# ricklisz/AnatoMask

Hardware: AMD Instinct MI355X
Metric: pretrain volumes/sec @128^3 patch mask=0.6 (higher is better)
Workload: dtype bf16; 1 GPU; STUNet-B AnatoMask step, 128^3 patch, mask_ratio 0.6, bf16 storage/MFMA + fp32 master; per_gpu_batch=16, global_batch=16, parallelism=dp1, step=teacher fwd + sampler + student fwd + loss + bwd + clip + AdamW + EMA

## Files before the change

### anatomask_amd/csrc/conv_igemm.hip

```cpp
#include <mutex>
#include <type_traits>
#include <stdlib.h>
#include "common.h"
#include "../../include/anatomask_hip.h"
#include "conv_plan.h"

using namespace amconv;

namespace {

template <typename T, int BD, int BH, int BW, int NS, int NIT, int TGS = 3, bool HR = false, bool NB = false, bool HT = false>
__global__ __launch_bounds__(256, (TGS == 2 && BD * BH * BW <= 256) ? 3 : 2) void conv_igemm_kernel(ConvArgs a) {
  constexpr int EPC = TT<T>::EPC;
  constexpr bool SPL = std::is_same<T, f32s_t>::value;
  constexpr int KC = (ROWB / 16) * EPC;
  constexpr int MV = BD * BH * BW;
  constexpr int VS = MV / 64;
  constexpr int NT = 16 * NS;
  constexpr int TG = TG_OF(NS, TGS);
  constexpr int WBUF = TG * NT * ROWB;
  constexpr int WCH = TG * NT * 4;
  constexpr int WIT = (WCH + 255) / 256;
  static_assert(MV % 64 == 0, "brick must give each wave whole 16-voxel subtiles");
  extern __shared__ __attribute__((aligned(16))) unsigned char lds[];
// ... 416 lines not shown
#pragma unroll
    for (int i = 0; i < NS; ++i)
#pragma unroll
      for (int r = 0; r < 4; ++r) {
        float s1 = 0.f, s2 = 0.f;
#pragma unroll
        for (int j = 0; j < VS; ++j) { const float o = acc[i][j][r]; s1 += o; s2 += o * o; }
        if (!AM_DBG(a, 2048)) { s1 = row16_sum(s1); s2 = row16_sum(s2); }
        if (r16 == 0) {
          const int c = (i >> 1) * 32 + g * 8 + (i & 1) * 4 + r;
          red[(wave * 16 * NS + c) * 2] = s1; red[(wave * 16 * NS + c) * 2 + 1] = s2;
        }
      }
    if (!AM_DBG(a, 1024)) __syncthreads();
    if (tid < 16 * NS && co0 + tid < a.Cout) {
      float s1 = 0.f, s2 = 0.f;
#pragma unroll
      for (int w = 0; w < 4; ++w) { s1 += red[(w * 16 * NS + tid) * 2]; s2 += red[(w * 16 * NS + tid) * 2 + 1]; }
      part[(co0 + tid) * 2] = s1; part[(co0 + tid) * 2 + 1] = s2;
    }
  }
}

template <typename T, int BD, int BH, int BW, int NS, int NIT, int TGS = 3, bool HR = false, bool NB = false, bool HT = false>
int launch(Plan& P, hipStream_t st) {
  ConvArgs& a = P.a;
  constexpr auto kern = conv_igemm_kernel<T, BD, BH, BW, NS, NIT, TGS, HR, NB, HT>;
  if (P.lds > 160 * 1024) return -3;
  AM_HIP_STAGE(am_lds_optin<kern>());
  const unsigned nbrick = a.plist ? (unsigned)a.nlive : (unsigned)(a.B * a.nbd * a.nbh * a.nbw);
  a.ny = (a.Cout + 16 * NS - 1) / (16 * NS);
  const unsigned nsib = (unsigned)(a.ny * a.nclass);
  dim3 grid(nsib > 1 ? ((nbrick + 7) / 8) * 8 * nsib : nbrick, 1, 1);
  AM_LAUNCH(kern, grid, dim3(256), P.lds, st, a);
  AM_CHECK_LAUNCH_STAGE();
  return 1;
}

template <typename T, int NS>
int dispatch_nit(Plan& P, int shape, hipStream_t st) {
  const int n = P.nit;
  if (P.a.nb_x) {
    if constexpr (sizeof(T) == 2) {
      if (P.tgs != 3 || P.a.OS != 1) return -7;
      if (shape == 2) return n <= 4 ? launch<T, 4, 4, 4, NS, 4, 3, false, true>(P, st) : -7;
      if (shape == 1) return n > 7 && n <= 11 ? (P.a.hreuse ? launch<T, 4, 4, 16, NS, 11, 3, true, true>(P, st) : launch<T, 4, 4, 16, NS, 11, 3, false, true>(P, st)) : -7;
// ... 54 lines not shown
  const int qd = (p.Do + os - 1) / os, qh = (p.Ho + os - 1) / os, qw = (p.Wo + os - 1) / os; const bool out_sparse = p.out_sparse;
  bool big_ok = p.dtype == AM_DT_BF16;
#ifdef AM_ABLATE
  { const char* e_ = getenv("AM_CV_NOBIG"); if (e_ && atoi(e_)) big_ok = false; }
#endif
  int shape = brick_shape(os, qh, qw, out_sparse, p.out_bshift, bd, bh, bw);
  *nt = Cout <= 32 ? 32 : 64;
  const long q = (long)qd * qh * qw;
  auto nwg = [&](int tile) { return (long)B * ((qd + *bd - 1) / *bd) * ((qh + *bh - 1) / *bh) * ((qw + *bw - 1) / *bw) * ((Cout + tile - 1) / tile) * (os == 2 ? 8 : 1); };
  if (nwg(*nt) < 256) {
    *nt = 32;
    if (nwg(32) < 192 && shape != 2) { shape = 2; *bh = 4; *bw = 4; }
  }
  if (os == 2 && !out_sparse && shape == 1 && *nt == 64 && qh >= 8 && nwg(64) >= 4096 && big_ok) { shape = 3; *bh = 8; }
  return shape;
}

extern "C" int am_packed_dims(int dtype, int rows, int k, int* rows_padded, int* k_padded) {
  const int tile = rows <= 32 ? 32 : 64;
  const int kc = dtype == AM_DT_BF16 ? 32 : 16;
  *rows_padded = (rows + tile - 1) / tile * tile;
  *k_padded = (k + kc - 1) / kc * kc;
  return 0;
}

int amconv::conv_igemm_fits(const ConvProblem& p) {
  const int os = p.mode == AM_CONV_DGRAD ? p.stride : (p.mode == AM_CONVT_FWD ? 2 : 1);
  int bd, bh, bw, nt;
  pick_tiling(p, &bd, &bh, &bw, &nt);
  return p.B * ((p.Do + os * bd - 1) / (os * bd)) * ((p.Ho + os * bh - 1) / (os * bh)) * ((p.Wo + os * bw - 1) / (os * bw)) * (os == 2 ? 8 : 1);
}

bool amconv::conv_igemm_serves(const ConvProblem& p) { return !p.prenorm; }

int amconv::conv_igemm_launch(const ConvProblem& p, ConvArgs& a0, const int* active_list, void* stream, int* rows) {
  if (!conv_igemm_serves(p)) return 0;
  Plan P;
  ConvArgs& a = P.a = a0;
  const int shape = pick_tiling(p, &P.bd, &P.bh, &P.bw, &P.nt_tile);
  const int rc = build_plan(P, p.mode, p.ksize, p.stride);
  if (rc) return rc;
  if (a.OS == 2 && p.accumulate && !p.partials && a.tap_begin[1] > a.tap_begin[0] && a.tap_begin[8] == a.tap_begin[1]) a.nclass = 1;
  if ((size_t)24 * p.Hi * p.Wi * p.Cin * 4 >= 0x7fffff00ull) return -5;
  const int Qd = (p.Do + a.OS - 1) / a.OS, Qh = (p.Ho + a.OS - 1) / a.OS, Qw = (p.Wo + a.OS - 1) / a.OS;
  a.nbd = (Qd + P.bd - 1) / P.bd; a.nbh = (Qh + P.bh - 1) / P.bh; a.nbw = (Qw + P.bw - 1) / P.bw;
  {
    const int qblock = p.out_sparse ? ((1 << p.out_bshift) / a.OS) : 0;
    a.brick_in_patch = qblock > 0 && qblock % P.bd == 0 && qblock % P.bh == 0 && qblock % P.bw == 0;
    bool listed = a.brick_in_patch && active_list && p.n_active > 0 && p.fd <= 255 && p.fh <= 255 && p.fw <= 255 && p.B <= 255 &&
                  Qd == p.fd * qblock && Qh == p.fh * qblock && Qw == p.fw * qblock;
#ifdef AM_ABLATE
    { const char* e = getenv("AM_CV_NOLIST"); if (e && atoi(e)) listed = false; }
#endif
    if (listed) {
      a.plist = active_list; a.pbd = qblock / P.bd; a.pbh = qblock / P.bh; a.pbw = qblock / P.bw;
      a.nlive = p.n_active * a.pbd * a.pbh * a.pbw;
    }
  }
  if (p.partials && p.dtype == AM_DT_BF16) {
    const size_t tile = (size_t)P.bd * P.bh * P.bw * (P.nt_tile * 2 + 32);
    if (P.lds < tile) P.lds = tile;
  }
  if (p.nbred) {
    const size_t tiles = (size_t)P.bd * P.bh * P.bw * (P.nt_tile * 4 + 32);
    if (P.lds < tiles) P.lds = tiles;
  }
  a.nt_store = ((size_t)p.B * p.Do * p.Ho * p.Wo * p.Cout * 2 >= ((size_t)384 << 20) && !p.accumulate) || AM_DBG(a, 8);
  hipStream_t st = (hipStream_t)stream;
  if (rows) *rows = (a.plist ? a.nlive : a.B * a.nbd * a.nbh * a.nbw) * a.nclass;
  return p.dtype == AM_DT_BF16 ? dispatch<bf16_t>(P, shape, st) : p.dtype == AM_DT_F32S ? dispatch<f32s_t>(P, shape, st) : dispatch<float>(P, shape, st);
}

#define AM_STAGE_ROW(name_) {#name_, name_##_fits, name_##_serves, name_##_launch}
static const ConvStage conv_stages[] = {AM_STAGE_ROW(conv_k3t), AM_STAGE_ROW(conv_k3), AM_STAGE_ROW(conv_rw), AM_STAGE_ROW(conv_gather), AM_STAGE_ROW(conv_igemm)};

static void query_masks(ConvProblem& p, bool sparse, int in_bshift, int out_bshift, int n_active) {
  p.in_sparse = p.out_sparse = sparse; p.same_mask = p.has_list = true;
  p.in_bshift = in_bshift; p.out_bshift = out_bshift; p.n_active = n_active;
}

extern "C" int am_conv3d_partials_rows(int mode, int dtype, int ksize, int stride, int B, int Do, int Ho, int Wo, int Cin, int Cout, int out_sparse,
                                       int out_bshift, int n_active, int* rows) {
  ConvProblem p{mode, dtype, ksize, stride, B, Do, Ho, Wo, Cin, Do, Ho, Wo, Cout};
  query_masks(p, out_sparse != 0, out_bshift, out_bshift, n_active);
  *rows = 0;
  for (const ConvStage& s : conv_stages) { const int r = s.fits(p); if (r > *rows) *rows = r; }
  return 0;
}

extern "C" int am_conv3d_uses_k3(int mode, int dtype, int ksize, int stride, int B, int Di, int Hi, int Wi, int Cin, int Do, int Ho, int Wo, int Cout,
                                 int has_masks, int accumulate, int fused_epilogue, int want_partials) {
  ConvProblem p{mode, dtype, ksize, stride, B, Di, Hi, Wi, Cin, Do, Ho, Wo, Cout};
  query_masks(p, has_masks != 0, 0, 0, 0);
  p.accumulate = accumulate != 0; p.ep = fused_epilogue != 0; p.partials = want_partials != 0;
  for (const ConvStage& s : conv_stages)
    if (s.serves(p)) return s.launch == conv_k3t_launch ? 2 : s.launch == conv_k3_launch ? 1 : 0;
  return 0;
}

static ConvArgs fill_args(const ConvProblem& p, const void* x, const void* w_packed, const float* bias, void* y, float* partials, const uint8_t* in_mask,
                          int in_bshift, const uint8_t* out_mask, int out_bshift, int fd, int fh, int fw, int accumulate) {
  ConvArgs a{};
  a.x = x; a.w = w_packed; a.bias = bias; a.y = y; a.partials = partials;
  a.B = p.B; a.Di = p.Di; a.Hi = p.Hi; a.Wi = p.Wi; a.Cin = p.Cin; a.Do = p.Do; a.Ho = p.Ho; a.Wo = p.Wo; a.Cout = p.Cout;
  am_packed_dims(p.dtype, p.Cout, p.Cin, &a.Coutp, &a.Cinp);
  a.w_bytes = p.ksize * p.ksize * p.ksize * a.Coutp * a.Cinp * (p.dtype == AM_DT_BF16 ? 2 : 4);
  a.in_mask = MaskView{in_mask, fd, fh, fw, in_bshift};
  a.out_mask = MaskView{out_mask, fd, fh, fw, out_bshift};
  a.accumulate = accumulate & 1; a.stats_sum_only = (accumulate & AM_CONV_PARTIALS_SUM_ONLY) ? 1 : 0;
#ifdef AM_ABLATE
  { const char* e = getenv("AM_CV_DBG"); a.dbg = e ? atoi(e) : 0; }
#endif
  return a;
}

static int conv3d_impl(ConvProblem& p, ConvArgs& a, const int* active_list, int n_active, void* stream, int* rows) {
  if (p.Cin % 8 || p.Cout % 8) return -1;
  p.in_sparse = a.in_mask.m != nullptr; p.out_sparse = a.out_mask.m != nullptr; p.same_mask = a.in_mask.m == a.out_mask.m;
  p.in_bshift = a.in_mask.bs; p.out_bshift = a.out_mask.bs; p.fd = a.in_mask.fd; p.fh = a.in_mask.fh; p.fw = a.in_mask.fw;
  p.has_list = active_list != nullptr; p.n_active = n_active;
  p.accumulate = a.accumulate != 0; p.sum_only = a.stats_sum_only != 0; p.partials = a.partials != nullptr;
  p.ep = a.ep_scale || a.ep_res || a.ep_act != AM_ACT_NONE; p.nbred = a.nb_x != nullptr; p.prenorm = a.in_scale != nullptr;
  for (const ConvStage& s : conv_stages) {
    const int rc = s.launch(p, a, active_list, stream, rows);
    if (rc) return rc == 1 ? 0 : rc;
  }
  return -7;
}

extern "C" int am_conv3d(int mode, int dtype, int ksize, int stride, const void* x, const void* w_packed,
                         const float* bias, void* y, int B, int Di, int Hi, int Wi, int Cin, int Do, int Ho, int Wo,
                         int Cout, const uint8_t* in_mask, int in_bshift, const uint8_t* out_mask, int out_bshift,
                         int fd, int fh, int fw, int accumulate, float* partials, const float* ep_scale, const float* ep_shift,
                         const void* ep_res, int ep_act, const int32_t* active_list, int n_active, int* partial_rows_written,
                         void* stream) {
  if (ep_scale && !ep_shift) return -1;
  ConvProblem p{mode, dtype, ksize, stride, B, Di, Hi, Wi, Cin, Do, Ho, Wo, Cout};
  ConvArgs a = fill_args(p, x, w_packed, bias, y, partials, in_mask, in_bshift, out_mask, out_bshift, fd, fh, fw, accumulate);
  a.ep_scale = ep_scale; a.ep_shift = ep_scale ? ep_shift : nullptr; a.ep_res = ep_res; a.ep_act = ep_act;
  return conv3d_impl(p, a, active_list, n_active, stream, partial_rows_written);
}

extern "C" int am_conv3d_prenorm_supported(int mode, int dtype, int ksize, int stride, int B, int Do, int Ho, int Wo, int Cin, int Cout,
                                           int sparse, int in_bshift, int out_bshift, int n_active) {
  if (!sparse) return 0;
// ... 8 lines not shown
                                 int out_bshift, int fd, int fh, int fw, float* partials, const float* in_scale, const float* in_shift,
                                 int in_act, const int32_t* active_list, int n_active, int* partial_rows_written, void* stream) {
  if (!in_scale || !in_shift || !mask || !active_list) return -1;
  if (in_act != AM_ACT_NONE && in_act != AM_ACT_LRELU && in_act != AM_ACT_RELU6) return -1;
  ConvProblem p{mode, dtype, ksize, stride, B, Di, Hi, Wi, Cin, Do, Ho, Wo, Cout};
  ConvArgs a = fill_args(p, x, w_packed, bias, y, partials, mask, in_bshift, mask, out_bshift, fd, fh, fw, 0);
  a.in_scale = in_scale; a.in_shift = in_shift; a.in_act = in_act;
  return conv3d_impl(p, a, active_list, n_active, stream, partial_rows_written);
}

extern "C" int am_conv3d_nbred(int mode, int dtype, int ksize, int stride, const void* x, const void* w_packed, void* y, int B, int Di,
                               int Hi, int Wi, int Cin, int Do, int Ho, int Wo, int Cout, const uint8_t* in_mask, int in_bshift,
                               const uint8_t* out_mask, int out_bshift, int fd, int fh, int fw, int accumulate, float* partials,
                               const void* nb_x, const float* nb_scale, const float* nb_shift, int nb_act,
                               int* partial_rows_written, void* stream) {
  if (dtype != AM_DT_BF16 || !partials || !nb_x) return -1;
  if (nb_act != AM_ACT_NONE && (!nb_scale || !nb_shift)) return -1;
  if (nb_act != AM_ACT_NONE && nb_act != AM_ACT_LRELU && nb_act != AM_ACT_RELU6) return -1;
  ConvProblem p{mode, dtype, ksize, stride, B, Di, Hi, Wi, Cin, Do, Ho, Wo, Cout};
  ConvArgs a = fill_args(p, x, w_packed, nullptr, y, partials, in_mask, in_bshift, out_mask, out_bshift, fd, fh, fw, accumulate);
  a.nb_x = nb_x; a.nb_scale = nb_scale; a.nb_shift = nb_shift; a.nb_act = nb_act;
  return conv3d_impl(p, a, nullptr, 0, stream, partial_rows_written);
}
```

### anatomask_amd/csrc/conv_plan.h

```cpp
#pragma once
#include "common.h"

namespace amconv {

struct ConvArgs {
  const void* x; const void* w; const float* bias; void* y; float* partials;
  const float* ep_scale; const float* ep_shift; const void* ep_res; int ep_act;
  const void* nb_x; const float* nb_scale; const float* nb_shift; int nb_act;
  const float* in_scale; const float* in_shift; int in_act;
  int B, Di, Hi, Wi, Cin, Do, Ho, Wo, Cout, Cinp, Coutp;
  int OS, GS, nclass, nunit;
  int ny;
  int nbd, nbh, nbw;
  int tap_begin[9];
  int upar[8];
  int taps[64];
  int mind[8], minh[8], minw[8];
  int ed[8], eh[8], ew[8];
  int mdiv_w[8], mdiv_hw[8];
  int w_bytes;
  int w_lds_off;
  MaskView in_mask, out_mask;
  int accumulate;
  int stats_sum_only;
  int brick_in_patch;
  const int* plist;
  int pbd, pbh, pbw, nlive;
  int hreuse;
  int nt_store;
#ifdef AM_ABLATE
  int dbg;
#endif
};

constexpr int ROWB = 64;
constexpr int LROWB = 80;
constexpr int TG_OF(int ns, int tgs) { return ns == 2 ? 2 * tgs : tgs; }

__device__ __forceinline__ int swz(int row, int chunk) { return (row << 6) + ((chunk ^ ((row >> 1) & 2)) << 4); }


enum TapRule { TAP_PLAIN, TAP_FLIPPED, TAP_SRC_PARITY, TAP_OUT_PARITY };
inline bool tap_shift(int rule, int t, int pad, int parity, int* u) {
  if (rule == TAP_PLAIN) { *u = t - pad; return true; }
  if (rule == TAP_FLIPPED) { *u = pad - t; return true; }
  if (rule == TAP_SRC_PARITY) { const int sft = t - pad, r = ((sft % 2) + 2) % 2; *u = (sft - r) / 2; return r == parity; }
  const int num = parity + pad - t; *u = num / 2; return !(num & 1);
}

struct Plan { ConvArgs a; int bd, bh, bw; size_t lds; int nit, nt_tile, tgs; };

inline int build_plan(Plan& P, int mode, int k, int stride) {
// ... 79 lines not shown
```

### anatomask_amd/engine.py

```python
from __future__ import annotations

from dataclasses import dataclass, field
from typing import Dict, List, Optional, Sequence, Tuple

import torch

from . import ops
from .ops import ACT_LRELU, ACT_NONE, ACT_RELU6, CONV_DGRAD, CONV_FWD, CONVT_DGRAD, CONVT_FWD, MaskInfo, NormStats

ENC = "sparse_encoder.sp_cnn.conv_blocks_context"
DEC = "dense_decoder.dec"


@dataclass
class Spec:
    dims: Sequence[int]
    depth: Sequence[int]
    width: int
    input_size: Tuple[int, int, int]
    in_ch: int = 1
    out_ch: int = 1
    downsample: int = 16
    n_stage: int = 5
    sync_bn: bool = False
# ... 486 lines not shown
    y2, a1, y1, out, x = t["y2"], t["a1"], t["y1"], t["out"], t["x"]
    dpre = torch.empty_like(y2)
    dy2 = ops.norm_backward(gout, out, y2, t["st2"], W[f"{p}.norm2.weight"], ACT_LRELU, mask, bs,
                            G[f"{p}.norm2.weight"], G[f"{p}.norm2.bias"], dres=dpre,
                            dbeta2=G.get(f"{p}.conv3.bias"), dxsum=G[f"{p}.conv2.bias"])
    sp = tuple(y2.shape[1:4])
    da1 = ops.conv3d(CONV_DGRAD, dy2, pk.get(W, f"{p}.conv2.weight", False, True), None, sp, 3, 1,
                     in_mask=mask, in_bshift=bs, out_mask=mask, out_bshift=bs)
    red1 = None
    _wgrad_into(pk, G, f"{p}.conv2.weight", CONV_FWD, a1, dy2, 3, 1, x_mask=mask, x_bshift=bs, y_mask=mask, y_bshift=bs)
    dy1 = ops.norm_backward(da1, None, y1, t["st1"], W[f"{p}.norm1.weight"], ACT_LRELU, mask, bs,
                            G[f"{p}.norm1.weight"], G[f"{p}.norm1.bias"], dxsum=G[f"{p}.conv1.bias"], reduced=red1)
    stride = t["stride"]
    if s == 0 and t["first"]:
        ops.stem_conv_wgrad(inp, dy1, 3, mask, bs, G[f"{p}.conv1.weight"].view(-1, 27), None, deterministic=pk.deterministic)
        ops.stem_conv_wgrad(inp, dpre, 1, mask, bs, G[f"{p}.conv3.weight"].view(-1, 1), None, deterministic=pk.deterministic)
        return None
    bsx = bs + (1 if stride == 2 else 0)
    spx = tuple(x.shape[1:4])
    _wgrad_into(pk, G, f"{p}.conv1.weight", CONV_FWD, x, dy1, 3, stride, x_mask=mask, x_bshift=bsx, y_mask=mask, y_bshift=bs)
    if free_saved:
        t["y1"] = t["a1"] = t["y2"] = t["out"] = None
    if t["first"]:
        gx = ops.conv3d(CONV_DGRAD, dy1, pk.get(W, f"{p}.conv1.weight", False, True), None, spx, 3, stride,
                        in_mask=mask, in_bshift=bs, out_mask=mask, out_bshift=bsx, out=base, accumulate=base is not None)
        _wgrad_into(pk, G, f"{p}.conv3.weight", CONV_FWD, x, dpre, 1, stride, x_mask=mask, x_bshift=bsx, y_mask=mask, y_bshift=bs)
        ops.conv3d(CONV_DGRAD, dpre, pk.get(W, f"{p}.conv3.weight", False, True), None, spx, 1, stride,
                   in_mask=mask, in_bshift=bs, out_mask=mask, out_bshift=bsx, out=gx, accumulate=True)
        return gx
    gx = ops.conv3d(CONV_DGRAD, dy1, pk.get(W, f"{p}.conv1.weight", False, True), None, spx, 3, 1,
                    in_mask=mask, in_bshift=bs, out_mask=mask, out_bshift=bs)
    return ops.add(gx, dpre, out=gx)


def encoder_backward(spec: Spec, W, G, pk: PackCache, inp: torch.Tensor, mask: MaskInfo, tape: Tape, dfeat, after_group=None):
    counts = tape.counts
    gstage: List[Optional[torch.Tensor]] = list(dfeat)
    by_stage: Dict[int, List[dict]] = {}
    for t in tape.enc:
        by_stage.setdefault(t["s"], []).append(t)
    for s in reversed(range(spec.n_stage)):
        if tape.recompute:
            xs, recs = tape.enc_in[s], []
            for b in range(spec.depth[s]):
                xs, r_ = _enc_block(W, pk, inp, mask, counts, spec.stage_spatial(s), s, b, xs)
                recs.append(r_)
# ... 82 lines not shown
```

### anatomask_amd/ops.py

```python
from __future__ import annotations

from typing import Optional, Tuple

import torch

from . import hip
from .hip import ACT_LRELU, ACT_NONE, ACT_RELU6, CONV_DGRAD, CONV_FWD, CONVT_DGRAD, CONVT_FWD


def _dt(t: torch.Tensor) -> int:
    if t.dtype == torch.float32:
        return hip.DT_F32
    if t.dtype == torch.bfloat16:
        return hip.DT_BF16
    raise TypeError(f"unsupported dtype {t.dtype}")


DEFAULT_F32_SPLIT = False


def _dtc(t: torch.Tensor, f32_split: bool) -> int:
    return hip.DT_F32S if (t.dtype == torch.float32 and f32_split) else _dt(t)


# ... 138 lines not shown
            assert taps <= 64
            blob += struct.pack("<QQqqiiiiii", w.data_ptr(), out.data_ptr(), sr, sk, R, K, taps, Rp, Kp, first)
            first += Rp * ((Kp + 63) // 64)
        self.n, self.blocks, self.dtype = len(pairs), first, dtype
        self.ptrs = [(w.data_ptr(), out.data_ptr()) for w, out in pairs]
        self.dev = torch.frombuffer(bytearray(blob), dtype=torch.uint8).to(device)

    def matches(self, pairs) -> bool:
        return len(pairs) == self.n and all(p == (w.data_ptr(), o.data_ptr()) for p, (w, o) in zip(self.ptrs, pairs))

    def repack(self):
        code = hip.DT_BF16 if self.dtype == torch.bfloat16 else (hip.DT_F32S if self.f32_split else hip.DT_F32)
        hip.lib().pack_weights_batched(code, self.dev.data_ptr(), self.n, self.blocks, _stream())


def unpack_grad(dw_packed: torch.Tensor, grad_out: torch.Tensor, transposed_conv: bool, accumulate: bool):
    taps, R, K = dw_packed.shape
    d1 = grad_out.shape[1]
    if transposed_conv:
        sr, sk = taps, d1 * taps
    else:
        sr, sk = d1 * taps, taps
    hip.lib().unpack_grad(dw_packed.data_ptr(), grad_out.data_ptr(), R, K, taps, sr, sk, int(accumulate), _stream())


def conv3d(mode: int, x: torch.Tensor, w_packed: torch.Tensor, bias: Optional[torch.Tensor], out_spatial: Tuple[int, int, int],
           ksize: int, stride: int, in_mask: Optional[MaskInfo] = None, in_bshift: int = 0,
           out_mask: Optional[MaskInfo] = None, out_bshift: int = 0, out: Optional[torch.Tensor] = None,
           accumulate: bool = False, want_partials: bool = False, ep_scale: Optional[torch.Tensor] = None,
           ep_shift: Optional[torch.Tensor] = None, ep_res: Optional[torch.Tensor] = None, ep_act: int = 0,
           norm_bwd: Optional[tuple] = None, partials_sum_only: bool = False):
    B, Di, Hi, Wi, Cin = x.shape
    Cout, Kl = w_packed.logical
    assert Kl == Cin and w_packed.dtype == x.dtype, (w_packed.logical, x.shape)
    Do, Ho, Wo = out_spatial
    mk = in_mask or out_mask
    mp, fd, fh, fw = _mk(mk)
    alp, aln = _al(out_mask) if (out_mask is not None and x.dtype == torch.bfloat16) else (None, 0)
    if norm_bwd is not None:
        xp, st, nact = norm_bwd
        assert x.dtype == torch.bfloat16 and xp.dtype == torch.bfloat16 and tuple(xp.shape) == (B, Do, Ho, Wo, Cout) and bias is None
        part = ConvPartials(mode, ksize, stride, B, out_spatial, Cout, x.device, out_mask is not None, out_bshift, _dt(x), 64, 0)
        if out is None:
            out = torch.empty(B, Do, Ho, Wo, Cout, device=x.device, dtype=x.dtype)
        hip.lib().conv3d_nbred(mode, _dt(x), ksize, stride, x.data_ptr(), w_packed.data_ptr(), out.data_ptr(),
                               B, Di, Hi, Wi, Cin, Do, Ho, Wo, Cout,
                               in_mask.t.data_ptr() if in_mask else None, in_bshift,
                               out_mask.t.data_ptr() if out_mask else None, out_bshift, fd, fh, fw, int(accumulate),
                               part.t.data_ptr(), xp.data_ptr(), st.scale.data_ptr(), st.shift.data_ptr(), int(nact), _ROWS_ADDR, _stream())
        part.rows = _ROWS_OUT.value
        return out, part
    split = _is_split(w_packed)
    part = ConvPartials(mode, ksize, stride, B, out_spatial, Cout, x.device, out_mask is not None, out_bshift, _dtc(x, split), Cin, aln) if want_partials else None
    if out is None:
        out = torch.empty(B, Do, Ho, Wo, Cout, device=x.device, dtype=x.dtype)
    rows = _ROWS_OUT
    hip.lib().conv3d(mode, _dtc(x, split), ksize, stride, x.data_ptr(), w_packed.data_ptr(), _p(bias), out.data_ptr(),
                     B, Di, Hi, Wi, Cin, Do, Ho, Wo, Cout,
                     in_mask.t.data_ptr() if in_mask else None, in_bshift,
                     out_mask.t.data_ptr() if out_mask else None, out_bshift, fd, fh, fw,
                     int(accumulate) | (2 if (partials_sum_only and part is not None) else 0),
                     part.t.data_ptr() if part else None, _p(ep_scale), _p(ep_shift),
                     ep_res.data_ptr() if ep_res is not None else None, int(ep_act), alp, aln, _ROWS_ADDR if part else None, _stream())
    if part is not None:
        part.rows = rows.value
        part.sum_only = bool(partials_sum_only)
    return (out, part) if want_partials else out


def conv3d_prenorm_supported(x: torch.Tensor, w_packed: torch.Tensor, out_spatial, ksize: int, stride: int, mask: Optional[MaskInfo], out_bshift: int) -> bool:
    if mask is None or x.dtype != torch.bfloat16 or _is_split(w_packed):
        return False
    lst, n = mask.active_list()
    if lst is None or n <= 0:
        return False
    Cout, Cin = w_packed.logical
    return hip.lib()._lib.am_conv3d_prenorm_supported(CONV_FWD, _dt(x), ksize, stride, x.shape[0], *out_spatial, Cin, Cout, 1,
                                                      out_bshift + (1 if stride == 2 else 0), out_bshift, n) == 1

# ... 463 lines not shown
```

### include/anatomask_hip.h

```cpp
#ifndef ANATOMASK_HIP_H
#define ANATOMASK_HIP_H
#include <stdint.h>
#ifdef __cplusplus
extern "C" {
#endif

#define AM_DT_F32 0
#define AM_DT_BF16 1
#define AM_DT_F32S 2

#define AM_CONV_PARTIALS_SUM_ONLY 2
#define AM_CONV_FWD 0
#define AM_CONV_DGRAD 1
#define AM_CONVT_FWD 2
#define AM_CONVT_DGRAD 3

#define AM_DXREP 64
#define AM_NREP 8

#define AM_ACT_NONE 0
#define AM_ACT_LRELU 1
#define AM_ACT_RELU6 2

int am_version(void);

int am_conv3d(int mode, int dtype, int ksize, int stride, const void* x, const void* w_packed, const float* bias, void* y,
              int B, int Di, int Hi, int Wi, int Cin, int Do, int Ho, int Wo, int Cout,
              const uint8_t* in_mask, int in_bshift, const uint8_t* out_mask, int out_bshift, int fd, int fh, int fw,
              int accumulate, float* partials ,
              const float* ep_scale, const float* ep_shift ,
              const void* ep_res ,
              int ep_act ,
              const int32_t* active_list, int n_active ,
              int* partial_rows_written ,
              void* stream);
int am_conv3d_prenorm_supported(int mode, int dtype, int ksize, int stride, int B, int Do, int Ho, int Wo, int Cin, int Cout, int sparse,
                                int in_bshift, int out_bshift, int n_active);
int am_conv3d_prenorm(int mode, int dtype, int ksize, int stride, const void* x, const void* w_packed, const float* bias, void* y, int B, int Di,
                      int Hi, int Wi, int Cin, int Do, int Ho, int Wo, int Cout, const uint8_t* mask, int in_bshift, int out_bshift, int fd,
                      int fh, int fw, float* partials , const float* in_scale, const float* in_shift, int in_act,
                      const int32_t* active_list, int n_active, int* partial_rows_written , void* stream);

int am_conv3d_nbred(int mode, int dtype, int ksize, int stride, const void* x, const void* w_packed, void* y, int B, int Di,
                    int Hi, int Wi, int Cin, int Do, int Ho, int Wo, int Cout, const uint8_t* in_mask, int in_bshift,
                    const uint8_t* out_mask, int out_bshift, int fd, int fh, int fw, int accumulate, float* partials,
                    const void* nb_x, const float* nb_scale, const float* nb_shift, int nb_act,
                    int* partial_rows_written, void* stream);
int am_packed_dims(int dtype, int rows, int k, int* rows_padded, int* k_padded);
int am_conv3d_partials_rows(int mode, int dtype, int ksize, int stride, int B, int Do, int Ho, int Wo, int Cin, int Cout,
                            int out_sparse, int out_bshift ,
                            int n_active, int* rows );
int am_conv3d_uses_k3(int mode, int dtype, int ksize, int stride, int B, int Di, int Hi, int Wi, int Cin, int Do, int Ho, int Wo, int Cout,
                      int has_masks, int accumulate, int fused_epilogue, int want_partials);
int am_partials_reduce(const float* partials, int rows, int C, double* sums, float* sum_accum, void* stream);

int am_conv3d_wgrad(int mode, int dtype, int ksize, int stride, const void* x, const void* dy, float* dw_packed,
                    int B, int Dx, int Hx, int Wx, int Cx, int Dy, int Hy, int Wy, int Cy,
                    const uint8_t* x_mask, int x_bshift, const uint8_t* y_mask, int y_bshift, int fd, int fh, int fw,
                    float* det_workspace, long det_workspace_floats,
                    const int32_t* active_list, int n_active ,
                    void* gather_workspace, long gather_workspace_bytes ,
                    void* stream);
int am_conv3d_wgrad_uses_k3(int mode, int dtype, int ksize, int stride, int B, int D, int H, int W, int Cx, int Cy, int has_masks,
                            int deterministic);
int am_conv3d_wgrad_gather_bytes(int mode, int dtype, int ksize, int stride, int B, int Cx, int Cy, int y_bshift, int has_y_mask, int n_active,
                                 int fd, int fh, int fw, long* bytes );

int am_split_bf16(const float* x, void* hi, void* lo, long n, void* stream);

int am_pack_weight(int dtype, const float* src, void* dst, int R, int K, int taps, long stride_r, long stride_k, int Rp, int Kp,
// ... 159 lines not shown
```

Measured before the change: 137.9 volumes/s.

## Add class-loop stride-2 dgrad kernel and fuse 1x1 shortcut dgrad into it

Adds a new implicit-GEMM kernel for stride-2 transposed and dgrad convolutions. Each workgroup stages the union input footprint for all 8 parity classes into LDS once and loops over the classes, instead of launching a separate brick per class that reloads overlapping input. A new pair entry point also folds the 1x1 stride-2 residual shortcut dgrad into the first class's accumulator, which removes a separate accumulate pass over the output. In exchange it brings larger LDS footprints, a longer serial loop per workgroup with less grid parallelism, and a fallback path when the plan does not qualify.

```diff
diff --git a/anatomask_amd/csrc/conv_igemm.hip b/anatomask_amd/csrc/conv_igemm.hip
--- a/anatomask_amd/csrc/conv_igemm.hip
+++ b/anatomask_amd/csrc/conv_igemm.hip
@@ -1,3 +1,4 @@
+#include <atomic>
 #include <mutex>
 #include <type_traits>
 #include <stdlib.h>
@@ -462,6 +463,355 @@
   }
 }
 
+template <typename T, int BD, int BH, int BW, int NS, int NIT>
+__global__ __launch_bounds__(256, 2) void conv_igemm_cl_kernel(ConvArgs a) {
+  constexpr int EPC = TT<T>::EPC;
+  constexpr bool SPL = std::is_same<T, f32s_t>::value;
+  constexpr int KC = (ROWB / 16) * EPC;
+  constexpr int MV = BD * BH * BW, VS = MV / 64, NT = 16 * NS, TG = TG_OF(NS, 2);
+  constexpr int WBUF = TG * NT * ROWB, WCH = TG * NT * 4, WIT = WCH / 256;
+  static_assert(MV % 64 == 0 && WCH % 256 == 0, "whole subtiles per wave, whole chunks per thread");
+  extern __shared__ __attribute__((aligned(16))) unsigned char lds[];
+  unsigned char* ldsW = lds + a.w_lds_off;
+
+  const int tid = threadIdx.x, lane = tid & 63, wave = tid >> 6;
+  const int g = lane >> 4, r16 = lane & 15;
+  const int nbrick = a.plist ? a.nlive : a.B * a.nbd * a.nbh * a.nbw;
+  int ytile = 0, bid = blockIdx.x;
+  if (a.ny > 1) {
+    const int t = bid >> 3;
+    ytile = t % a.ny;
+    bid = ((t / a.ny) << 3) + (bid & 7);
+    if (bid >= nbrick) return;
+  }
+  const int brick = bid;
+  int bw_, bh_, bd_, b;
+  if (a.plist) {
+    const int bpp = a.pbd * a.pbh * a.pbw;
+    const int pk = a.plist[bid / bpp], j = bid % bpp;
+    b = (pk >> 24) & 255;
+    bd_ = ((pk >> 16) & 255) * a.pbd + j / (a.pbh * a.pbw); bh_ = ((pk >> 8) & 255) * a.pbh + (j / a.pbw) % a.pbh; bw_ = (pk & 255) * a.pbw + j % a.pbw;
+  } else {
+    bw_ = bid % a.nbw; bid /= a.nbw;
+    bh_ = bid % a.nbh; bid /= a.nbh;
+    bd_ = bid % a.nbd; b = bid / a.nbd;
+  }
+  const int q0d = bd_ * BD, q0h = bh_ * BH, q0w = bw_ * BW;
+  const int co0 = ytile * NT;
+  float* part0 = a.partials ? a.partials + (size_t)brick * a.Cout * 2 : nullptr;
+  const size_t part_cls = (size_t)nbrick * a.Cout * 2;
+
+  if (!a.plist && a.out_mask.m) {
+    bool live;
+    if (a.brick_in_patch) live = a.out_mask.active(b, q0d * 2, q0h * 2, q0w * 2);
+    else {
+      int any = 0;
+      for (int v = tid; v < MV; v += 256) {
+        const int od = (q0d + v / (BW * BH)) * 2, oh = (q0h + (v / BW) % BH) * 2, ow = (q0w + v % BW) * 2;
+        if (od < a.Do && oh < a.Ho && ow < a.Wo && a.out_mask.active(b, od, oh, ow)) any = 1;
+      }
+      live = __syncthreads_or(any) != 0;
+    }
+    if (!live) {
+      if (part0 && tid < NT && co0 + tid < a.Cout)
+        for (int c = 0; c < 8; ++c) { part0[c * part_cls + (co0 + tid) * 2] = 0.f; part0[c * part_cls + (co0 + tid) * 2 + 1] = 0.f; }
+      return;
+    }
+  }
+
+  int tapv;
+  {
+    const int tp = a.taps[lane];
+    const int ud = (tp & 15) - 8, uh = ((tp >> 4) & 15) - 8, uw = ((tp >> 8) & 15) - 8;
+    tapv = ((((ud - a.cl_mind) * a.cl_eh + (uh - a.cl_minh)) * a.cl_ew + (uw - a.cl_minw)) * LROWB) | (((tp >> 12) & 63) << 20);
+  }
+  const size_t plane_elems = (size_t)a.Hi * a.Wi * a.Cin;
+  const __amdgpu_buffer_rsrc_t rw = __builtin_amdgcn_make_buffer_rsrc((void*)a.w, 0, a.w_bytes, 0x00020000);
+  constexpr unsigned OOB = 0x80000000u;
+  const int cchunk = (tid & 3) * EPC;
+  const int sdst = (tid >> 2) * LROWB + (tid & 3) * (SPL ? 8 : 16);
+  const int wtapB = a.Coutp * a.Cinp * (int)sizeof(T);
+  const int nslab = a.Cinp / KC;
+
+  unsigned wsrc[WIT];
+  int wdst[WIT];
+#pragma unroll
+  for (int it = 0; it < WIT; ++it) {
+    const int idx = tid + it * 256;
+    const int row = (idx >> 2) % NT, tig = idx / (NT * 4);
+    wsrc[it] = (unsigned)(((co0 + crow(row)) * a.Cinp + (idx & 3) * EPC) * (int)sizeof(T));
+    wdst[it] = tig * NT * ROWB + swz(row, idx & 3);
+  }
+  int aoff[NS];
+#pragma unroll
+  for (int i = 0; i < NS; ++i) aoff[i] = swz(i * 16 + r16, g);
+
+#define AM_CL_WLOAD(WR, TB, NTP, GI, KCW, OK)                                                               \
+  _Pragma("unroll") for (int it = 0; it < WIT; ++it) {                                                      \
+    const int tt_ = __builtin_amdgcn_readfirstlane((GI) * TG + (tid + it * 256) / (NT * 4));                \
+    const int wi_ = __builtin_amdgcn_readlane(tapv, (TB) + (tt_ < (NTP) ? tt_ : (NTP) - 1)) >> 20;          \
+    WR[it] = __builtin_bit_cast(u32x4, __builtin_amdgcn_raw_buffer_load_b128(rw, (tt_ < (NTP) && (OK)) ? wsrc[it] : OOB, wi_ * wtapB + (KCW) * (int)sizeof(T), 0)); \
+  }
+#define AM_CL_WSTORE(WR, BUF)                                                                              \
+  _Pragma("unroll") for (int it = 0; it < WIT; ++it)                                                        \
+    *(u32x4*)(ldsW + (BUF) * WBUF + wdst[it]) = WR[it];
+
+  u32x4 wr[WIT];
+  AM_CL_WLOAD(wr, a.tap_begin[0], a.tap_begin[1] - a.tap_begin[0], 0, 0, true);
+
+  u32x4 xa[2][NS], xb[2][VS];
+  auto x2_load = [&](const int s, const int h) __attribute__((always_inline)) {
+    const int kc = s * KC + g * EPC;
+    const bool sok = s < nslab;
+    const u32x4 z4 = {0u, 0u, 0u, 0u};
+#pragma unroll
+    for (int i = 0; i < NS; ++i)
+      xa[h][i] = sok ? *(const u32x4*)((const T*)a.w2 + (size_t)(co0 + crow(i * 16 + r16)) * a.Cinp + kc) : z4;
+#pragma unroll
+    for (int j = 0; j < VS; ++j) {
+      const int v = wave * (MV / 4) + j * 16 + r16;
+      const int qd = q0d + v / (BW * BH), qh = q0h + (v / BW) % BH, qw = q0w + v % BW;
+      const bool ok = sok && qd < a.Di && qh < a.Hi && qw < a.Wi && kc < a.Cin;
+      xb[h][j] = ok ? *(const u32x4*)((const T*)a.x2 + (((size_t)(b * a.Di + qd) * a.Hi + qh) * a.Wi + qw) * a.Cin + kc) : z4;
+    }
+  };
+  auto x2_mma = [&](f32x4 (&acc_)[NS][VS], const int h) __attribute__((always_inline)) {
+    if constexpr (!SPL) {
+#pragma unroll
+      for (int j = 0; j < VS; ++j)
+#pragma unroll
+        for (int i = 0; i < NS; ++i) acc_[i][j] = mma_chunk<T>(xa[h][i], xb[h][j], acc_[i][j]);
+    }
+  };
+  if constexpr (!SPL) {
+    if (a.x2) { x2_load(0, 0); x2_load(1, 1); }
+  }
+
+  {
+    const int ED = a.cl_ed, EH = a.cl_eh, EW = a.cl_ew, nvox = ED * EH * EW, EHW = EH * EW;
+    const int i0d = q0d + a.cl_mind, i0h = q0h + a.cl_minh, i0w = q0w + a.cl_minw;
+    int dbase = i0d < 0 ? 0 : (i0d > a.Di ? a.Di : i0d);
+    const size_t left = (size_t)(a.Di - dbase) * plane_elems * sizeof(T);
+    const __amdgpu_buffer_rsrc_t rx = __builtin_amdgcn_make_buffer_rsrc(
+        (void*)((const T*)a.x + ((size_t)b * a.Di + dbase) * plane_elems), 0, (int)(left < 0x7fffff00ull ? left : 0x7fffff00ull), 0x00020000);
+    unsigned soff[NIT];
+    uint8_t mb[NIT];
+#pragma unroll
+    for (int it = 0; it < NIT; ++it) {
+      const int e = (tid + it * 256) >> 2;
+      const int ez = (e * a.cl_mdiv_hw) >> 20, rem = e - ez * EHW;
+      const int ey = (rem * a.cl_mdiv_w) >> 20, ex = rem - ey * EW;
+      const int id = i0d + ez, ih = i0h + ey, iw = i0w + ex;
+      const bool ok = e < nvox && (unsigned)id < (unsigned)a.Di && (unsigned)ih < (unsigned)a.Hi && (unsigned)iw < (unsigned)a.Wi;
+      soff[it] = ok ? (unsigned)(((((id - dbase) * a.Hi + ih) * a.Wi + iw) * a.Cin + cchunk) * (int)sizeof(T)) : OOB;
+      mb[it] = a.in_mask.m ? a.in_mask.peek(b, id, ih, iw, ok) : (uint8_t)1;
+    }
+#pragma unroll
+    for (int it = 0; it < NIT; ++it)
+      if (!mb[it]) soff[it] = OOB;
+    for (int s0 = 0; s0 < nslab; s0 += 2) {
+      u32x4 stg[2][NIT];
+#pragma unroll
+      for (int h = 0; h < 2; ++h) {
+        const bool cok = (s0 + h) * KC + cchunk < a.Cin && s0 + h < nslab;
+#pragma unroll
+        for (int it = 0; it < NIT; ++it)
+          stg[h][it] = __builtin_bit_cast(u32x4, __builtin_amdgcn_raw_buffer_load_b128(rx, cok ? soff[it] : OOB, (s0 + h) * KC * (int)sizeof(T), 0));
+      }
+#pragma unroll
+      for (int h = 0; h < 2; ++h)
+        if (s0 + h < nslab) {
+          unsigned char* dsl = lds + (s0 + h) * a.cl_slab + sdst;
+#pragma unroll
+          for (int it = 0; it < NIT; ++it)
+            if (((tid + it * 256) >> 2) < nvox) {
+              if constexpr (SPL) {
+                typedef __attribute__((ext_vector_type(2))) unsigned int u32x2_;
+                unsigned h2[2], l2[2];
+                split4_bf16(stg[h][it], h2, l2);
+                *(u32x2_*)(dsl + it * 64 * LROWB) = u32x2_{h2[0], h2[1]};
+                *(u32x2_*)(dsl + it * 64 * LROWB + 32) = u32x2_{l2[0], l2[1]};
+              } else {
+                *(u32x4*)(dsl + it * 64 * LROWB) = stg[h][it];
+              }
+            }
+        }
+    }
+  }
+  AM_CL_WSTORE(wr, 0);
+  __syncthreads();
+
+  int bb[VS];
+#pragma unroll
+  for (int j = 0; j < VS; ++j) {
+    const int v = wave * (MV / 4) + j * 16 + r16;
+    bb[j] = (((v / (BW * BH)) * a.cl_eh + (v / BW) % BH) * a.cl_ew + v % BW) * LROWB + (SPL ? (g & 1) : g) * 16;
+  }
+  T* __restrict__ yg = (T*)a.y;
+  constexpr int NH = NS / 2;
+  f32x4 bia[NS];
+#pragma unroll
+  for (int i = 0; i < NS; ++i) {
+    const int co = co0 + (i >> 1) * 32 + g * 8 + (i & 1) * 4;
+    bia[i] = (a.bias && co < a.Cout) ? *(const f32x4*)(a.bias + co) : f32x4{0.f, 0.f, 0.f, 0.f};
+  }
+  const bool sparse_out = a.out_mask.m != nullptr;
+  auto load8 = [&](const T* p, f32x4& lo, f32x4& hi) {
+    if constexpr (sizeof(T) == 4) { lo = *(const f32x4*)p; hi = *(const f32x4*)(p + 4); }
+    else {
+      typedef __attribute__((ext_vector_type(8))) __bf16 bfx8_;
+      typedef __attribute__((ext_vector_type(8))) float f32x8_;
+      const f32x8_ f = __builtin_convertvector(*(const bfx8_*)p, f32x8_);
+      lo = f32x4{f[0], f[1], f[2], f[3]}; hi = f32x4{f[4], f[5], f[6], f[7]};
+    }
+  };
+
+  int bufp = 0;
+  for (int cls = 0; cls < 8; ++cls) {
+    const int tb = a.tap_begin[cls], nt = a.tap_begin[cls + 1] - tb, ng = (nt + TG - 1) / TG;
+    const int tbn = a.tap_begin[cls < 7 ? cls + 1 : cls], ntn = a.tap_begin[cls < 7 ? cls + 2 : cls + 1] - tbn;
+    const int pd = (cls >> 2) & 1, ph = (cls >> 1) & 1, pw = cls & 1;
+    f32x4 acc[NS][VS];
+#pragma unroll
+    for (int i = 0; i < NS; ++i)
+#pragma unroll
+      for (int j = 0; j < VS; ++j) acc[i][j] = f32x4{0.f, 0.f, 0.f, 0.f};
+
+    if constexpr (!SPL) {
+      if (cls == 0 && a.x2) {
+#pragma unroll
+        for (int h = 0; h < 2; ++h) {
+          x2_mma(acc, h);
+          x2_load(2 + h, h);
+        }
+      }
+    }
+
+    for (int s = 0; s < nslab; ++s) {
+      const unsigned char* slab = lds + s * a.cl_slab;
+      for (int gi = 0; gi < ng; ++gi) {
+        const bool more_g = gi + 1 < ng, more_s = s + 1 < nslab;
+        const bool same = more_g || more_s;
+        AM_CL_WLOAD(wr, same ? tb : tbn, same ? nt : ntn, more_g ? gi + 1 : 0, more_g ? s * KC : (more_s ? (s + 1) * KC : 0), same || cls < 7);
+        __builtin_amdgcn_sched_barrier(0);
+        __builtin_amdgcn_s_setprio(1);
+#pragma unroll
+        for (int tl = 0; tl < TG; ++tl) {
+          const int tt = gi * TG + tl;
+          const int tob = __builtin_amdgcn_readlane(tapv, tb + (tt < nt ? tt : nt - 1)) & 0xFFFFF;
+          u32x4 af[NS];
+#pragma unroll
+          for (int i = 0; i < NS; ++i) af[i] = *(const u32x4*)(ldsW + bufp * WBUF + tl * NT * ROWB + aoff[i]);
+#pragma unroll
+          for (int j = 0; j < VS; ++j) {
+            const u32x4 bf = *(const u32x4*)(slab + bb[j] + tob);
+            if constexpr (SPL) {
+              const u32x4 bf2 = *(const u32x4*)(slab + bb[j] + tob + 32);
+#pragma unroll
+              for (int i = 0; i < NS; ++i) acc[i][j] = mma_split(af[i], bf, bf2, acc[i][j]);
+            } else {
+#pragma unroll
+              for (int i = 0; i < NS; ++i) acc[i][j] = mma_chunk<T>(af[i], bf, acc[i][j]);
+            }
+          }
+        }
+        __builtin_amdgcn_s_setprio(0);
+        __builtin_amdgcn_sched_barrier(0);
+        AM_CL_WSTORE(wr, bufp ^ 1);
+        __syncthreads();
+        bufp ^= 1;
+      }
+    }
+
+    if constexpr (!SPL) {
+      if (cls == 0 && a.x2 && nslab > 2) { x2_mma(acc, 0); x2_mma(acc, 1); }
+    }
+
+#pragma unroll
+    for (int j = 0; j < VS; ++j) {
+      const int v = wave * (MV / 4) + j * 16 + r16;
+      const int od = (q0d + v / (BW * BH)) * 2 + pd, oh = (q0h + (v / BW) % BH) * 2 + ph, ow = (q0w + v % BW) * 2 + pw;
+      const bool inr = od < a.Do && oh < a.Ho && ow < a.Wo;
+      const bool act = inr && (!sparse_out || a.out_mask.active(b, od, oh, ow));
+      const size_t ovox = ((size_t)(b * a.Do + od) * a.Ho + oh) * a.Wo + ow;
+      T* dstv = yg + ovox * a.Cout + co0 + g * 8;
+#pragma unroll
+      for (int h = 0; h < NH; ++h) {
+        f32x4 o0 = acc[2 * h][j] + bia[2 * h], o1 = acc[2 * h + 1][j] + bia[2 * h + 1];
+        T* dst = dstv + h * 32;
+        const bool wrt = inr && co0 + h * 32 + g * 8 < a.Cout;
+        if (sparse_out && !act) { o0 = f32x4{0.f, 0.f, 0.f, 0.f}; o1 = o0; }
+        if (a.accumulate && act && wrt) {
+          f32x4 p0_, p1_;
+          load8(dst, p0_, p1_);
+          o0 += p0_; o1 += p1_;
+        }
+        if constexpr (sizeof(T) == 4) {
+          if (wrt) { *(f32x4*)dst = o0; *(f32x4*)(dst + 4) = o1; }
+          acc[2 * h][j] = act && wrt ? o0 : f32x4{0.f, 0.f, 0.f, 0.f};
+          acc[2 * h + 1][j] = act && wrt ? o1 : f32x4{0.f, 0.f, 0.f, 0.f};
+        } else {
+          typedef __attribute__((ext_vector_type(4))) __bf16 bfx4;
+          typedef __attribute__((ext_vector_type(8))) __bf16 bfx8;
+          const bfx4 p0 = __builtin_convertvector(o0, bfx4), p1 = __builtin_convertvector(o1, bfx4);
+          if (wrt) { if (a.nt_store) __builtin_nontemporal_store(__builtin_shufflevector(p0, p1, 0, 1, 2, 3, 4, 5, 6, 7), (bfx8*)dst); else *(bfx8*)dst = __builtin_shufflevector(p0, p1, 0, 1, 2, 3, 4, 5, 6, 7); }
+        }
+      }
+    }
+    if constexpr (sizeof(T) == 4) {
+      if (part0) {
+        float* part = part0 + cls * part_cls;
+        float* red = (float*)(lds + a.cl_red_off);
+#pragma unroll
+        for (int i = 0; i < NS; ++i)
+#pragma unroll
+          for (int r = 0; r < 4; ++r) {
+            float s1 = 0.f, s2 = 0.f;
+#pragma unroll
+            for (int j = 0; j < VS; ++j) { const float o = acc[i][j][r]; s1 += o; s2 += o * o; }
+            s1 = row16_sum(s1); s2 = row16_sum(s2);
+            if (r16 == 0) {
+              const int c = (i >> 1) * 32 + g * 8 + (i & 1) * 4 + r;
+              red[(wave * 16 * NS + c) * 2] = s1; red[(wave * 16 * NS + c) * 2 + 1] = s2;
+            }
+          }
+        __syncthreads();
+        if (tid < 16 * NS && co0 + tid < a.Cout) {
+          float s1 = 0.f, s2 = 0.f;
+#pragma unroll
+          for (int w = 0; w < 4; ++w) { s1 += red[(w * 16 * NS + tid) * 2]; s2 += red[(w * 16 * NS + tid) * 2 + 1]; }
+          part[(co0 + tid) * 2] = s1; part[(co0 + tid) * 2 + 1] = s2;
+        }
+      }
+    }
+  }
+#undef AM_CL_WLOAD
+#undef AM_CL_WSTORE
+}
+
+std::atomic<int> g_class_loop{1};
+std::atomic<int> g_class_loop_launches{0};
+
+template <typename T, int BD, int BH, int BW, int NS, int NIT>
+int launch_cl(Plan& P, hipStream_t st) {
+  ConvArgs& a = P.a;
+  constexpr auto kern = conv_igemm_cl_kernel<T, BD, BH, BW, NS, NIT>;
+  AM_HIP_STAGE(am_lds_optin<kern>());
+  const unsigned nbrick = a.plist ? (unsigned)a.nlive : (unsigned)(a.B * a.nbd * a.nbh * a.nbw);
+  dim3 grid(a.ny > 1 ? ((nbrick + 7) / 8) * 8 * a.ny : nbrick, 1, 1);
+  AM_LAUNCH(kern, grid, dim3(256), P.lds, st, a);
+  AM_CHECK_LAUNCH_STAGE();
+  g_class_loop_launches.fetch_add(1, std::memory_order_relaxed);
+  return 1;
+}
+
+template <typename T, int NS>
+int dispatch_cl(Plan& P, int shape, hipStream_t st) {
+  const int n = P.nit;
+  if (shape == 1) return n <= 7 ? launch_cl<T, 4, 4, 16, NS, 7>(P, st) : launch_cl<T, 4, 4, 16, NS, 11>(P, st);
+  return n <= 7 ? launch_cl<T, 4, 8, 8, NS, 7>(P, st) : launch_cl<T, 4, 8, 8, NS, 11>(P, st);
+}
+
 template <typename T, int BD, int BH, int BW, int NS, int NIT, int TGS = 3, bool HR = false, bool NB = false, bool HT = false>
 int launch(Plan& P, hipStream_t st) {
   ConvArgs& a = P.a;
@@ -562,6 +912,40 @@
   *rows_padded = (rows + tile - 1) / tile * tile;
   *k_padded = (k + kc - 1) / kc * kc;
   return 0;
+}
+
+constexpr int AM_CL_MIN_WG_PER_CU = 1;
+constexpr size_t AM_CL_MAX_LDS = 80 * 1024;
+static bool class_loop_plan(const ConvProblem& p, Plan& P, int shape) {
+  ConvArgs& a = P.a;
+  const int mode = g_class_loop.load(std::memory_order_relaxed);
+  if (!mode || a.OS != 2 || a.nclass != 8 || shape > 1) return false;
+  if (p.ep || p.nbred || (p.partials && p.dtype == AM_DT_BF16) || (p.out_sparse && a.out_mask.bs < 1)) return false;
+  if (a.x2 && (p.dtype == AM_DT_F32S || p.partials || a.Cinp / (p.dtype == AM_DT_BF16 ? 32 : 16) > 4)) return false;
+  if (a.x2 && a.in_mask.m && (a.in_mask.m != a.out_mask.m || a.in_mask.bs + 1 != a.out_mask.bs)) return false;
+  int mn[3] = {a.mind[0], a.minh[0], a.minw[0]}, mx[3] = {mn[0], mn[1], mn[2]};
+  for (int c = 0; c < 8; ++c) {
+    if (a.tap_begin[c + 1] == a.tap_begin[c]) return false;
+    const int lo[3] = {a.mind[c], a.minh[c], a.minw[c]}, hi[3] = {a.mind[c] + a.ed[c] - P.bd, a.minh[c] + a.eh[c] - P.bh, a.minw[c] + a.ew[c] - P.bw};
+    for (int d = 0; d < 3; ++d) { if (lo[d] < mn[d]) mn[d] = lo[d]; if (hi[d] > mx[d]) mx[d] = hi[d]; }
+  }
+  a.cl_mind = mn[0]; a.cl_minh = mn[1]; a.cl_minw = mn[2];
+  a.cl_ed = P.bd + mx[0] - mn[0]; a.cl_eh = P.bh + mx[1] - mn[1]; a.cl_ew = P.bw + mx[2] - mn[2];
+  a.cl_mdiv_w = (1 << 20) / a.cl_ew + 1;
+  a.cl_mdiv_hw = (1 << 20) / (a.cl_ew * a.cl_eh) + 1;
+  const int nvox = a.cl_ed * a.cl_eh * a.cl_ew, nit = (nvox * (ROWB / 16) + 255) / 256;
+  if (nit > 11) return false;
+  a.cl_slab = nvox * LROWB;
+  const int nslab = a.Cinp / (p.dtype == AM_DT_BF16 ? 32 : 16);
+  const size_t w_off = (size_t)nslab * a.cl_slab, red_off = w_off + 2 * TG_OF(P.nt_tile / 16, 2) * P.nt_tile * ROWB;
+  const size_t lds = red_off + (p.partials ? 4 * P.nt_tile * 2 * sizeof(float) : 0);
+  if (lds > 160 * 1024 || (mode == 1 && lds > AM_CL_MAX_LDS)) return false;
+  const int ny = (a.Cout + P.nt_tile - 1) / P.nt_tile;
+  const long nbrick = a.plist ? a.nlive : (long)a.B * a.nbd * a.nbh * a.nbw;
+  if (mode == 1 && nbrick * ny < (long)AM_CL_MIN_WG_PER_CU * am_cu_count()) return false;
+  a.w_lds_off = (int)w_off; a.cl_red_off = (int)red_off;
+  P.nit = nit; P.lds = lds; a.ny = ny;
+  return true;
 }
 
 int amconv::conv_igemm_fits(const ConvProblem& p) {
@@ -608,6 +992,11 @@
   a.nt_store = ((size_t)p.B * p.Do * p.Ho * p.Wo * p.Cout * 2 >= ((size_t)384 << 20) && !p.accumulate) || AM_DBG(a, 8);
   hipStream_t st = (hipStream_t)stream;
   if (rows) *rows = (a.plist ? a.nlive : a.B * a.nbd * a.nbh * a.nbw) * a.nclass;
+  if (class_loop_plan(p, P, shape))
+    return p.dtype == AM_DT_BF16 ? (P.nt_tile == 32 ? dispatch_cl<bf16_t, 2>(P, shape, st) : dispatch_cl<bf16_t, 4>(P, shape, st))
+         : p.dtype == AM_DT_F32S ? (P.nt_tile == 32 ? dispatch_cl<f32s_t, 2>(P, shape, st) : dispatch_cl<f32s_t, 4>(P, shape, st))
+                                 : (P.nt_tile == 32 ? dispatch_cl<float, 2>(P, shape, st) : dispatch_cl<float, 4>(P, shape, st));
+  if (a.x2) return 0;
   return p.dtype == AM_DT_BF16 ? dispatch<bf16_t>(P, shape, st) : p.dtype == AM_DT_F32S ? dispatch<f32s_t>(P, shape, st) : dispatch<float>(P, shape, st);
 }
 
@@ -654,13 +1043,17 @@
   return a;
 }
 
-static int conv3d_impl(ConvProblem& p, ConvArgs& a, const int* active_list, int n_active, void* stream, int* rows) {
-  if (p.Cin % 8 || p.Cout % 8) return -1;
+static void fill_problem(ConvProblem& p, const ConvArgs& a, const int* active_list, int n_active) {
   p.in_sparse = a.in_mask.m != nullptr; p.out_sparse = a.out_mask.m != nullptr; p.same_mask = a.in_mask.m == a.out_mask.m;
   p.in_bshift = a.in_mask.bs; p.out_bshift = a.out_mask.bs; p.fd = a.in_mask.fd; p.fh = a.in_mask.fh; p.fw = a.in_mask.fw;
   p.has_list = active_list != nullptr; p.n_active = n_active;
   p.accumulate = a.accumulate != 0; p.sum_only = a.stats_sum_only != 0; p.partials = a.partials != nullptr;
   p.ep = a.ep_scale || a.ep_res || a.ep_act != AM_ACT_NONE; p.nbred = a.nb_x != nullptr; p.prenorm = a.in_scale != nullptr;
+}
+
+static int conv3d_impl(ConvProblem& p, ConvArgs& a, const int* active_list, int n_active, void* stream, int* rows) {
+  if (p.Cin % 8 || p.Cout % 8) return -1;
+  fill_problem(p, a, active_list, n_active);
   for (const ConvStage& s : conv_stages) {
     const int rc = s.launch(p, a, active_list, stream, rows);
     if (rc) return rc == 1 ? 0 : rc;
@@ -715,3 +1108,34 @@
   a.nb_x = nb_x; a.nb_scale = nb_scale; a.nb_shift = nb_shift; a.nb_act = nb_act;
   return conv3d_impl(p, a, nullptr, 0, stream, partial_rows_written);
 }
+
+extern "C" int am_conv3d_s2_dgrad_pair(int dtype, const void* x, const void* w_packed, const void* x2, const void* w2_packed, void* y, int B,
+                                       int Di, int Hi, int Wi, int Cin, int Do, int Ho, int Wo, int Cout, const uint8_t* in_mask, int in_bshift,
+                                       const uint8_t* out_mask, int out_bshift, int fd, int fh, int fw, int accumulate,
+                                       const int32_t* active_list, int n_active, void* stream) {
+  if (!x2 || !w2_packed) return -1;
+  if (Cin % 8 || Cout % 8) return -1;
+  ConvProblem p{AM_CONV_DGRAD, dtype, 3, 2, B, Di, Hi, Wi, Cin, Do, Ho, Wo, Cout};
+  ConvArgs a = fill_args(p, x, w_packed, nullptr, y, nullptr, in_mask, in_bshift, out_mask, out_bshift, fd, fh, fw, accumulate & 1);
+  fill_problem(p, a, active_list, n_active);
+  bool earlier = false;
+  for (const ConvStage& s : conv_stages) { if (s.launch == conv_igemm_launch) break; if (s.serves(p)) earlier = true; }
+  if (!earlier) {
+    a.x2 = x2; a.w2 = w2_packed;
+    const int rc = conv_igemm_launch(p, a, active_list, stream, nullptr);
+    if (rc) return rc == 1 ? 0 : rc;
+    a.x2 = a.w2 = nullptr;
+  }
+  const int rc = conv3d_impl(p, a, active_list, n_active, stream, nullptr);
+  if (rc) return rc;
+  ConvProblem p1{AM_CONV_DGRAD, dtype, 1, 2, B, Di, Hi, Wi, Cin, Do, Ho, Wo, Cout};
+  ConvArgs a1 = fill_args(p1, x2, w2_packed, nullptr, y, nullptr, in_mask, in_bshift, out_mask, out_bshift, fd, fh, fw, 1);
+  return conv3d_impl(p1, a1, active_list, n_active, stream, nullptr);
+}
+
+extern "C" int am_set_s2_class_loop(int on) {
+  if (on < 0 || on > 2) return -1;
+  g_class_loop.store(on, std::memory_order_relaxed);
+  return 0;
+}
+extern "C" int am_s2_class_loop_launches(int* n) { if (!n) return -1; *n = g_class_loop_launches.load(std::memory_order_relaxed); return 0; }
diff --git a/anatomask_amd/csrc/conv_plan.h b/anatomask_amd/csrc/conv_plan.h
--- a/anatomask_amd/csrc/conv_plan.h
+++ b/anatomask_amd/csrc/conv_plan.h
@@ -28,6 +28,10 @@
   int pbd, pbh, pbw, nlive;
   int hreuse;
   int nt_store;
+  int cl_mind, cl_minh, cl_minw, cl_ed, cl_eh, cl_ew, cl_mdiv_w, cl_mdiv_hw;
+  int cl_slab;
+  int cl_red_off;
+  const void* x2; const void* w2;
 #ifdef AM_ABLATE
   int dbg;
 #endif
diff --git a/anatomask_amd/engine.py b/anatomask_amd/engine.py
--- a/anatomask_amd/engine.py
+++ b/anatomask_amd/engine.py
@@ -532,6 +532,10 @@
     if free_saved:
         t["y1"] = t["a1"] = t["y2"] = t["out"] = None
     if t["first"]:
+        if stride == 2:
+            _wgrad_into(pk, G, f"{p}.conv3.weight", CONV_FWD, x, dpre, 1, stride, x_mask=mask, x_bshift=bsx, y_mask=mask, y_bshift=bs)
+            return ops.conv3d_s2_dgrad_pair(dy1, pk.get(W, f"{p}.conv1.weight", False, True), dpre, pk.get(W, f"{p}.conv3.weight", False, True),
+                                            spx, in_mask=mask, in_bshift=bs, out_mask=mask, out_bshift=bsx, out=base, accumulate=base is not None)
         gx = ops.conv3d(CONV_DGRAD, dy1, pk.get(W, f"{p}.conv1.weight", False, True), None, spx, 3, stride,
                         in_mask=mask, in_bshift=bs, out_mask=mask, out_bshift=bsx, out=base, accumulate=base is not None)
         _wgrad_into(pk, G, f"{p}.conv3.weight", CONV_FWD, x, dpre, 1, stride, x_mask=mask, x_bshift=bsx, y_mask=mask, y_bshift=bs)
diff --git a/anatomask_amd/ops.py b/anatomask_amd/ops.py
--- a/anatomask_amd/ops.py
+++ b/anatomask_amd/ops.py
@@ -184,6 +184,42 @@
     else:
         sr, sk = d1 * taps, taps
     hip.lib().unpack_grad(dw_packed.data_ptr(), grad_out.data_ptr(), R, K, taps, sr, sk, int(accumulate), _stream())
+
+
+S2_CLASS_LOOP = True
+_S2_PUSHED = None
+
+
+def _push_s2_switch():
+    global _S2_PUSHED
+    if int(S2_CLASS_LOOP) != _S2_PUSHED:
+        _S2_PUSHED = int(S2_CLASS_LOOP)
+        hip.lib().set_s2_class_loop(_S2_PUSHED)
+
+
+def s2_class_loop_launches() -> int:
+    n = _ct.c_int(0)
+    hip.lib().s2_class_loop_launches(_ct.addressof(n))
+    return n.value
+
+
+def conv3d_s2_dgrad_pair(x: torch.Tensor, w_packed: torch.Tensor, x2: torch.Tensor, w2_packed: torch.Tensor, out_spatial: Tuple[int, int, int],
+                         in_mask: Optional[MaskInfo] = None, in_bshift: int = 0, out_mask: Optional[MaskInfo] = None, out_bshift: int = 0,
+                         out: Optional[torch.Tensor] = None, accumulate: bool = False) -> torch.Tensor:
+    B, Di, Hi, Wi, Cin = x.shape
+    Cout, Kl = w_packed.logical
+    assert Kl == Cin and tuple(w2_packed.logical) == (Cout, Cin) and x2.shape == x.shape and x2.dtype == x.dtype
+    assert w_packed.dtype == x.dtype and w2_packed.dtype == x.dtype and _is_split(w_packed) == _is_split(w2_packed)
+    Do, Ho, Wo = out_spatial
+    mp, fd, fh, fw = _mk(in_mask or out_mask)
+    alp, aln = _al(out_mask) if (out_mask is not None and x.dtype == torch.bfloat16) else (None, 0)
+    if out is None:
+        out = torch.empty(B, Do, Ho, Wo, Cout, device=x.device, dtype=x.dtype)
+    _push_s2_switch()
+    hip.lib().conv3d_s2_dgrad_pair(_dtc(x, _is_split(w_packed)), x.data_ptr(), w_packed.data_ptr(), x2.data_ptr(), w2_packed.data_ptr(), out.data_ptr(),
+                                   B, Di, Hi, Wi, Cin, Do, Ho, Wo, Cout, in_mask.t.data_ptr() if in_mask else None, in_bshift,
+                                   out_mask.t.data_ptr() if out_mask else None, out_bshift, fd, fh, fw, int(accumulate), alp, aln, _stream())
+    return out
 
 
 def conv3d(mode: int, x: torch.Tensor, w_packed: torch.Tensor, bias: Optional[torch.Tensor], out_spatial: Tuple[int, int, int],
@@ -217,6 +253,7 @@
     if out is None:
         out = torch.empty(B, Do, Ho, Wo, Cout, device=x.device, dtype=x.dtype)
     rows = _ROWS_OUT
+    _push_s2_switch()
     hip.lib().conv3d(mode, _dtc(x, split), ksize, stride, x.data_ptr(), w_packed.data_ptr(), _p(bias), out.data_ptr(),
                      B, Di, Hi, Wi, Cin, Do, Ho, Wo, Cout,
                      in_mask.t.data_ptr() if in_mask else None, in_bshift,
diff --git a/include/anatomask_hip.h b/include/anatomask_hip.h
--- a/include/anatomask_hip.h
+++ b/include/anatomask_hip.h
@@ -46,6 +46,12 @@
                     const uint8_t* out_mask, int out_bshift, int fd, int fh, int fw, int accumulate, float* partials,
                     const void* nb_x, const float* nb_scale, const float* nb_shift, int nb_act,
                     int* partial_rows_written, void* stream);
+int am_conv3d_s2_dgrad_pair(int dtype, const void* x, const void* w_packed, const void* x2, const void* w2_packed, void* y, int B,
+                            int Di, int Hi, int Wi, int Cin, int Do, int Ho, int Wo, int Cout, const uint8_t* in_mask, int in_bshift,
+                            const uint8_t* out_mask, int out_bshift, int fd, int fh, int fw, int accumulate ,
+                            const int32_t* active_list, int n_active, void* stream);
+int am_set_s2_class_loop(int on);
+int am_s2_class_loop_launches(int* n);
 int am_packed_dims(int dtype, int rows, int k, int* rows_padded, int* k_padded);
 int am_conv3d_partials_rows(int mode, int dtype, int ksize, int stride, int B, int Do, int Ho, int Wo, int Cin, int Cout,
                             int out_sparse, int out_bshift ,
```

After: 138.0 volumes/s (median of 3 runs). Within noise of the previous version (+0.1%).
